# zertovitch/zip-ada

Hardware: AMD Instinct MI355X
Metric: Deflate encode MB/s (Deflate_3; stream bit-exact with the CPU restatement of the reference, Ada parity unpinned) (higher is better)
Workload: dtype u8

## Files before the change

### zip-ada_amd/csrc/zada_huff.hip

```cpp
#include <hip/hip_runtime.h>
#include <stdlib.h>
#include <stdio.h>
#include <stdint.h>
#include "zada_logic.h"
#include "zada_descr_bound.h"
#include "zada_internal.h"
#include "zada_llhc_wave.h"

namespace zada {

__device__ __forceinline__ void atom_symbols(uint32_t t, int &ls, int &ds) {
  if (tok_is_match(t)) { ls = len_symbol((int)((t >> 16) & 0x1FF)); ds = dist_symbol((int)(t & 0xFFFF)); }
  else { ls = (int)(t & 0xFF); ds = -1; }
}

__device__ __forceinline__ void put_bits_global(uint32_t *out32, uint64_t pos, uint32_t value, int nbits) {
  if (nbits <= 0) return;
  uint64_t w = pos >> 5; int sh = (int)(pos & 31);
  uint64_t v = (uint64_t)value << sh;
  atomicOr(&out32[w], (uint32_t)v);
  if (sh + nbits > 32) atomicOr(&out32[w + 1], (uint32_t)(v >> 32));
}

__device__ __forceinline__ void put_bits_lim(uint32_t *out32, uint64_t lim_bits, uint64_t pos, uint32_t value, int nbits) {
// ... 721 lines not shown
      const ChRec r = chrec[i];
      uint64_t rb = INF;
      if (T == BT_FIXED) rb = r.bits[0];
      else if (T == BT_DYNAMIC) {
        if (code_block == (int)i - 1) { if ((r.ok >> code_variant) & 1u) rb = r.bits[code_variant]; }
        else {
          const BlockInfo *bi = &binfo[i];
          const uint8_t *cl = code_block == CODE_CARRIED ? cin->bl : (code_variant == 1 ? binfo[code_block].bl1 : binfo[code_block].bl2);
          bool bad = false; uint64_t rc = 0;
          for (int q = 0; q < 5; q++) {
            const int s = lane + 64 * q;
            const int cu = cl[s]; const uint32_t stv = bi->stats[s];
            if (cu == 0 && bi->bl1[s] > 0) bad = true;
            if (s < 288) { if (s != 256 && s <= 285) rc += (uint64_t)stv * (uint64_t)(cu + litlen_sym_extra(s)); }
            else if (s - 288 <= 29) rc += (uint64_t)stv * (uint64_t)(cu + dist_sym_extra(s - 288));
          }
          rc = wave_sum_u64(rc);
          if (!__any(bad)) rb = rc;
        }
      }
      const bool finishing = B && (T == BT_FIXED || T == BT_DYNAMIC);
      const uint64_t c = 1 + (finishing ? (uint64_t)(eob >> 16) : 0);
      dec = ch_decide(r, c, rb);
      if (lane == 0) {
        ChW w; w.rdata = rb; w.eob_in = eob; w.dec = (uint8_t)dec; w.T_in = (uint8_t)T; w.B_in = (uint8_t)B; w.pad = 0;
        w.code_block = code_block; w.code_variant = (uint32_t)code_variant; w.npieces = 0; w.bytes_pad = 0;
        chw[i] = w;
      }
    } else dec = chw[i].dec;
    if (dec != FMT_RECYCLE) {
      uint32_t j = nblocks;
      for (uint32_t b0 = i + 1; b0 < nblocks && j == nblocks; b0 += 64) {
        const uint32_t k = b0 + (uint32_t)lane;
        const bool rcy = k < nblocks && chw[k].dec == FMT_RECYCLE;
        const unsigned long long m = __ballot(rcy);
        if (m) j = b0 + (uint32_t)(__ffsll((long long)m) - 1);
      }
      if (j == nblocks) break;
      out_state(j - 1);
      i = j; need_eval = false;
    } else {
      i++; need_eval = true;
    }
  }
}

template <typename F>
__device__ __forceinline__ uint32_t ch_stored_walk(const uint32_t *__restrict__ apos, uint32_t first, uint32_t count, uint32_t end_byte, int last_block, F &&piece) {
  uint32_t stk_first[40], stk_last[40]; int stk_lb[40]; int sp = 0;
  uint32_t np = 0;
  stk_first[0] = first; stk_last[0] = first + count - 1; stk_lb[0] = last_block; sp = 1;
  while (sp > 0) {
    sp--;
    const uint32_t f = stk_first[sp], l = stk_last[sp]; const int lb = stk_lb[sp];
    const uint32_t src = apos[f], nbytes = ((end_byte && l + 1 == first + count) ? end_byte : apos[l + 1]) - src;
    if (nbytes > 0xFFFF) {
      const uint32_t mid = (uint32_t)(((uint64_t)f + (uint64_t)l) / 2);
      stk_first[sp] = mid + 1; stk_last[sp] = l; stk_lb[sp] = lb; sp++;
      stk_first[sp] = f; stk_last[sp] = mid; stk_lb[sp] = 0; sp++;
      continue;
    }
    piece(np, src, nbytes, lb);
    np++;
  }
  return np;
}

__global__ void __launch_bounds__(64) k_ch_stored(uint32_t nblocks, const ChRec *__restrict__ chrec, const uint32_t *__restrict__ apos, ChW *__restrict__ chw) {
  const uint32_t i = blockIdx.x * blockDim.x + threadIdx.x;
  if (i >= nblocks || chw[i].dec != FMT_STORED) return;
  const BlockRange br = chrec[i].br;
  chw[i].npieces = ch_stored_walk(apos, br.first, br.count, br.pad, (int)(br.last_flush & BR_LAST_FLUSH), [](uint32_t, uint32_t, uint32_t, int) {});
}

struct PosFn { uint64_t a, b; uint32_t kind; };
__device__ __forceinline__ uint64_t posfn_apply(const PosFn &f, uint64_t p) { return f.kind == 2 ? f.b : f.kind ? ((p + f.a + 7) & ~7ull) + f.b : p + f.a; }
__device__ __forceinline__ PosFn posfn_compose(const PosFn &f, const PosFn &g) {
  PosFn h;
  if (g.kind == 2) return g;
  if (f.kind == 2) { h.kind = 2; h.a = 0; h.b = posfn_apply(g, f.b); return h; }
  if (g.kind == 0) { h.kind = f.kind; h.a = f.kind ? f.a : f.a + g.a; h.b = f.kind ? f.b + g.a : 0; }
  else if (f.kind == 0) { h.kind = 1; h.a = f.a + g.a; h.b = g.b; }
  else { h.kind = 1; h.a = f.a; h.b = ((f.b + g.a + 7) & ~7ull) + g.b; }
  return h;
}

__global__ void __launch_bounds__(1024) k_ch_layout(uint32_t nblocks, const ChRec *__restrict__ chrec, const BlockInfo *__restrict__ binfo, const ChW *__restrict__ chw,
                                                    EmitRec *__restrict__ emit, uint32_t *__restrict__ piece_base, uint32_t cap_tiles, uint32_t cap_pieces,
                                                    uint32_t *__restrict__ out32, uint64_t lim_bits, ChooserOut *__restrict__ res,
                                                    const ChooserCarry *__restrict__ cin, ChooserCarry *__restrict__ cout, uint64_t base_bits, int do_epilogue,
                                                    const uint32_t *__restrict__ blk_entry, EntOut *__restrict__ ent_out ) {
  __shared__ PosFn wfn[16];
  __shared__ uint32_t wtiles[16], wpieces[16], wlast[16];
  __shared__ uint64_t s_pos; __shared__ uint32_t s_tiles, s_pieces, s_last;
  const int tid = threadIdx.x, lane = tid & 63, w = tid >> 6;
  if (tid == 0) { s_pos = cin->pos - base_bits; s_tiles = 0; s_pieces = 0; s_last = 0xFFFFFFFFu; }
  __syncthreads();
  for (uint32_t t0 = 0; t0 < nblocks; t0 += 1024) {
    const uint32_t i = t0 + (uint32_t)tid;
    const bool ex = i < nblocks;
    PosFn f; f.kind = 0; f.a = 0; f.b = 0;
    uint32_t nt = 0, np = 0, opener = 0xFFFFFFFFu;
    ChRec r; ChW cw;
    uint64_t pre_bits = 0, hdr = 0, data = 0, opt = 0;
    bool opens = false;
    if (ex) {
      r = chrec[i]; cw = chw[i];
      const bool fin = cw.B_in && (cw.T_in == BT_FIXED || cw.T_in == BT_DYNAMIC);
      const uint64_t eobl = fin ? (uint64_t)(cw.eob_in >> 16) : 0;
      const uint64_t c = 1 + eobl;
      if (cw.dec == FMT_STORED) {
        np = cw.npieces;
        f.kind = 1; f.a = eobl + 3; f.b = 32ull * np + 8ull * (np - 1) + 8ull * binfo[i].bytes;
        opt = r.stored + c; opener = i;
      } else {
        nt = (r.br.count + TILE - 1) / TILE;
        if (cw.dec == FMT_RECYCLE) { data = cw.rdata; opt = cw.rdata; }
        else if (cw.dec == FMT_FIXED) { opens = cw.T_in != BT_FIXED; data = r.fixed_data; opt = r.base3 + c; }
        else { opens = true; hdr = cw.dec == FMT_DYN1 ? r.hdr1 : r.hdr2; data = cw.dec == FMT_DYN1 ? r.dyn1_data : r.dyn2_data; opt = r.base3 + c; }
        if (opens) { pre_bits = eobl + 3; opener = i; }
        f.a = pre_bits + hdr + data;
      }
    }
    const bool efirst = ex && ent_out && (r.br.last_flush & BR_ENTRY_FIRST), elast = ex && ent_out && (r.br.last_flush & BR_ENTRY_LAST);
    const PosFn fown = f;
    if (efirst) { f.kind = 2; f.a = 0; f.b = posfn_apply(fown, 0); }
    PosFn inc = f; uint32_t it = nt, ip = np, il = opener;
    for (int off = 1; off < 64; off <<= 1) {
      PosFn o; o.a = __shfl_up(inc.a, off); o.b = __shfl_up(inc.b, off); o.kind = __shfl_up(inc.kind, off);
      const uint32_t ot = __shfl_up(it, off), op = __shfl_up(ip, off), ol = __shfl_up(il, off);
      if (lane >= off) { inc = posfn_compose(o, inc); it += ot; ip += op; il = il == 0xFFFFFFFFu ? ol : il; }
    }
    if (lane == 63) { wfn[w] = inc; wtiles[w] = it; wpieces[w] = ip; }
    {
      const unsigned long long m = __ballot(opener != 0xFFFFFFFFu);
      if (lane == 0) wlast[w] = m ? t0 + (uint32_t)(w * 64 + 63 - __builtin_clzll(m)) : 0xFFFFFFFFu;
    }
    __syncthreads();
    PosFn before; before.kind = 0; before.a = 0; before.b = 0;
    uint32_t tb = 0, pb = 0;
    for (int k = 0; k < w; k++) { before = posfn_compose(before, wfn[k]); tb += wtiles[k]; pb += wpieces[k]; }
    PosFn exl; exl.a = __shfl_up(inc.a, 1); exl.b = __shfl_up(inc.b, 1); exl.kind = __shfl_up(inc.kind, 1);
    uint32_t ext = __shfl_up(it, 1), exp_ = __shfl_up(ip, 1);
    if (lane == 0) { exl.kind = 0; exl.a = 0; exl.b = 0; ext = 0; exp_ = 0; }
    const PosFn upto = posfn_compose(before, exl);
    const uint64_t p0 = efirst ? 0 : posfn_apply(upto, s_pos);
    const uint32_t tile0 = s_tiles + tb + ext, piece0 = s_pieces + pb + exp_;
    if (ex) {
      EmitRec e; e.hdr_bitpos = 0; e.data_bitpos = 0; e.cost_bits = opt; e.fmt = cw.dec; e.code_block = CODE_FIXED; e.code_variant = 0; e.tile_base = tile0;
      e.pre_pos = 0; e.pre_eob = 0; e.pre_flags = 0;
      if (cw.dec == FMT_STORED) {
        e.pre_pos = p0;
        e.pre_eob = (cw.B_in && (cw.T_in == BT_FIXED || cw.T_in == BT_DYNAMIC)) ? cw.eob_in : 0u;
        piece_base[i] = piece0;
      } else {
        if (opens) {
          e.pre_pos = p0;
          e.pre_eob = (cw.B_in && (cw.T_in == BT_FIXED || cw.T_in == BT_DYNAMIC)) ? cw.eob_in : 0u;
          e.pre_flags = 1u | ((r.br.last_flush & BR_LAST_FLUSH) << 1) | ((cw.dec == FMT_FIXED ? 1u : 2u) << 2);
        }
        e.hdr_bitpos = p0 + pre_bits;
        e.data_bitpos = p0 + pre_bits + hdr;
        if (cw.dec == FMT_RECYCLE || (cw.dec == FMT_FIXED && !opens)) { e.code_block = cw.code_block; e.code_variant = cw.code_variant; }
        else if (cw.dec == FMT_FIXED) { e.code_block = CODE_FIXED; e.code_variant = 0; }
        else { e.code_block = (int32_t)i; e.code_variant = cw.dec == FMT_DYN1 ? 1u : 2u; }
      }
      emit[i] = e;
      if (elast) {
        uint32_t lo = il;
        if (lo == 0xFFFFFFFFu) { for (int k = w - 1; k >= 0; k--) if (wlast[k] != 0xFFFFFFFFu) { lo = wlast[k]; break; } }
        if (lo == 0xFFFFFFFFu) lo = s_last;
        const uint32_t dk = chw[lo].dec;
        const ChRec rk = chrec[lo];
        EntOut eo; eo.bits = posfn_apply(fown, p0);
        eo.eob = dk == FMT_STORED ? 0u : dk == FMT_FIXED ? (7u << 16) : rk.eob[dk == FMT_DYN1 ? 0 : 1];
        eo.fake = (rk.br.last_flush & BR_LAST_FLUSH) ? 0u : 1u;
        ent_out[blk_entry[i]] = eo;
      }
    }
    __syncthreads();
    if (tid == 1023) {
      const PosFn all = posfn_compose(before, inc);
      s_pos = posfn_apply(all, s_pos); s_tiles += tb + it; s_pieces += pb + ip;
    }
    if (tid == 0) { for (int k = 15; k >= 0; k--) if (wlast[k] != 0xFFFFFFFFu) { s_last = wlast[k]; break; } }
    __syncthreads();
  }
  uint64_t pos = s_pos;
  int T = cin->last_type, B = cin->block_to_finish, M = cin->last_marked;
  uint32_t eob = cin->cur_eob;
  const uint8_t *cl = T == BT_DYNAMIC ? cin->bl : nullptr;
  if (s_last != 0xFFFFFFFFu) {
    const uint32_t k = s_last;
    const uint32_t dec = chw[k].dec;
    const ChRec r = chrec[k];
    B = 1; M = (int)(r.br.last_flush & BR_LAST_FLUSH); cl = nullptr;
    if (dec == FMT_STORED) T = BT_STORED;
    else if (dec == FMT_FIXED) { T = BT_FIXED; eob = 7u << 16; }
    else { T = BT_DYNAMIC; eob = r.eob[dec == FMT_DYN1 ? 0 : 1]; cl = dec == FMT_DYN1 ? binfo[k].bl1 : binfo[k].bl2; }
    if (dec == FMT_STORED) eob = chw[k].eob_in;
  }
  if (do_epilogue) {
    if (B && (T == BT_FIXED || T == BT_DYNAMIC)) {
      if (tid == 0) put_bits_lim(out32, lim_bits, pos, eob & 0xFFFF, (int)(eob >> 16));
      pos += (uint64_t)(eob >> 16);
    }
    if (!M) {
      if (tid == 0) { put_bits_lim(out32, lim_bits, pos, 1, 1); put_bits_lim(out32, lim_bits, pos + 1, 1, 2); }
      pos += 3 + 7;
    }
  }
  if (tid < 320) cout->bl[tid] = cl ? cl[tid] : (uint8_t)0;
  if (tid == 0) {
    res->total_bits = pos; res->n_tiles = s_tiles; res->n_pieces = s_pieces; res->n_blocks = nblocks;
    res->overflow = (s_tiles > cap_tiles || s_pieces > cap_pieces) ? 1u : 0u;
    cout->pos = pos + base_bits; cout->last_type = T; cout->block_to_finish = B; cout->last_marked = M; cout->cur_eob = eob; cout->pad[0] = cout->pad[1] = 0;
  }
}

__global__ void k_batch_geom(uint32_t E, const uint32_t *__restrict__ chunk0, const uint32_t *__restrict__ fl0, const uint32_t *__restrict__ ent_start,
                             const uint32_t *__restrict__ ent_len, const uint32_t *__restrict__ offsets, const uint32_t *__restrict__ total_atoms,
                             FlushGeom *__restrict__ ftab, EntOut *__restrict__ ent_out) {
  const uint32_t e = blockIdx.x * blockDim.x + threadIdx.x;
  if (e >= E) return;
  const uint32_t a0 = offsets[chunk0[e]], a1 = e + 1 < E ? offsets[chunk0[e + 1]] : *total_atoms, T = a1 - a0;
  const uint32_t nfl = (T + FLUSH - 1) / FLUSH;
  for (uint32_t s = fl0[e], k = 0; s < fl0[e + 1]; s++, k++) {
    FlushGeom g; g.F = a0 + k * FLUSH; g.to = 0; g.gj = k; g.flags = FG_EMPTY; g.end_byte = ent_start[e] + ent_len[e]; g.entry = e; g.pad[0] = g.pad[1] = 0;
    if (k < nfl) {
      g.to = g.F + FLUSH - 1 < a1 - 1 ? g.F + FLUSH - 1 : a1 - 1;
      g.flags = (k == 0 ? (uint32_t)FG_ENTRY_FIRST : 0u) | (k + 1 == nfl ? (uint32_t)FG_ENTRY_LAST : 0u) |
                ((k + 1 == nfl && (T % FLUSH) != 0) ? (uint32_t)FG_LAST_PARTIAL : 0u);
    }
    ftab[s] = g;
  }
  EntOut eo; eo.bits = 0; eo.eob = 0; eo.fake = 1;
  ent_out[e] = eo;
}

__global__ void k_batch_sizes(uint32_t E, const EntOut *__restrict__ ent_out, uint32_t *__restrict__ ent_bytes) {
  const uint32_t e = blockIdx.x * blockDim.x + threadIdx.x;
  if (e >= E) return;
  const EntOut eo = ent_out[e];
  ent_bytes[e] = (uint32_t)((eo.bits + (eo.eob >> 16) + (eo.fake ? 10u : 0u) + 7) / 8);
}

__global__ void k_batch_rebase(uint32_t nblocks, const uint32_t *__restrict__ blk_entry, const uint32_t *__restrict__ ent_base, EmitRec *__restrict__ emit) {
  const uint32_t i = blockIdx.x * blockDim.x + threadIdx.x;
  if (i >= nblocks) return;
  const uint64_t b = 8ull * ent_base[blk_entry[i]];
  emit[i].hdr_bitpos += b; emit[i].data_bitpos += b; emit[i].pre_pos += b;
}

__global__ void k_batch_finish(uint32_t E, const EntOut *__restrict__ ent_out, const uint32_t *__restrict__ ent_base, uint32_t *__restrict__ out32, uint64_t lim_bits) {
  const uint32_t e = blockIdx.x * blockDim.x + threadIdx.x;
  if (e >= E) return;
  const EntOut eo = ent_out[e];
  uint64_t pos = 8ull * ent_base[e] + eo.bits;
  if (eo.eob) { put_bits_lim(out32, lim_bits, pos, eo.eob & 0xFFFF, (int)(eo.eob >> 16)); pos += eo.eob >> 16; }
  if (eo.fake) { put_bits_lim(out32, lim_bits, pos, 1, 1); put_bits_lim(out32, lim_bits, pos + 1, 1, 2); }
}

__global__ void __launch_bounds__(64) k_ch_stored_emit(uint32_t nblocks, const ChRec *__restrict__ chrec, const ChW *__restrict__ chw, const EmitRec *__restrict__ emit,
                                                       const uint32_t *__restrict__ piece_base, const uint32_t *__restrict__ apos,
                                                       StoredPiece *__restrict__ pieces, uint32_t *__restrict__ out32, uint64_t lim_bits) {
  const uint32_t i = blockIdx.x * blockDim.x + threadIdx.x;
  if (i >= nblocks || chw[i].dec != FMT_STORED) return;
  const BlockRange br = chrec[i].br;
  const EmitRec e = emit[i];
  uint64_t pos = e.pre_pos;
  const uint32_t pb = piece_base[i];
  bool first = true;
  ch_stored_walk(apos, br.first, br.count, br.pad, (int)(br.last_flush & BR_LAST_FLUSH), [&](uint32_t k, uint32_t src, uint32_t nbytes, int lb) {
    if (first && e.pre_eob) { put_bits_lim(out32, lim_bits, pos, e.pre_eob & 0xFFFF, (int)(e.pre_eob >> 16)); pos += e.pre_eob >> 16; }
    first = false;
    put_bits_lim(out32, lim_bits, pos, (uint32_t)lb, 1);
    pos += 3;
    pos = (pos + 7) & ~7ull;
    put_bits_lim(out32, lim_bits, pos, nbytes & 0xFFFF, 16);
    put_bits_lim(out32, lim_bits, pos + 16, (~nbytes) & 0xFFFF, 16);
    StoredPiece pc; pc.dst_byte = (pos >> 3) + 4; pc.src_byte = src; pc.nbytes = nbytes;
    pieces[pb + k] = pc;
    pos += 32 + 8ull * nbytes;
  });
}

__global__ void __launch_bounds__(256) k_emit_prefix(uint32_t nblocks, const EmitRec *__restrict__ emit, const BlockRange *__restrict__ blocks,
                                                     uint32_t *__restrict__ tile_block, uint32_t *__restrict__ out32) {
  const uint32_t i = blockIdx.x * blockDim.x + threadIdx.x;
  if (i >= nblocks) return;
  const EmitRec e = emit[i];
  if (e.pre_flags & 1u) {
    uint64_t p = e.pre_pos;
    if (e.pre_eob) { put_bits_global(out32, p, e.pre_eob & 0xFFFF, (int)(e.pre_eob >> 16)); p += e.pre_eob >> 16; }
    put_bits_global(out32, p, (e.pre_flags >> 1) & 1u, 1);
    put_bits_global(out32, p + 1, (e.pre_flags >> 2) & 3u, 2);
  }
  if (e.fmt != FMT_STORED) {
    const uint32_t nt = (blocks[i].count + TILE - 1) / TILE;
    for (uint32_t t = 0; t < nt; t++) tile_block[e.tile_base + t] = i;
  }
}

__global__ void __launch_bounds__(64) k_block_codes(uint32_t nblocks, const EmitRec *__restrict__ emit, const BlockInfo *__restrict__ binfo,
                                                    uint32_t *__restrict__ codes, const ChooserCarry *__restrict__ cin) {
  __shared__ uint8_t bl[320];
  __shared__ uint16_t cd[320];
  const uint32_t b = blockIdx.x;
  const int lane = threadIdx.x;
  if (b == nblocks) {
    for (int i = lane; i < 320; i += 64) bl[i] = (uint8_t)(i < 288 ? fixed_litlen_bl(i) : 5);
  } else if (b == nblocks + 1) {
    for (int i = lane; i < 320; i += 64) bl[i] = cin->bl[i];
  } else {
    const uint32_t f = emit[b].fmt;
    if (f != FMT_DYN1 && f != FMT_DYN2) return;
    const uint8_t *src = f == FMT_DYN1 ? binfo[b].bl1 : binfo[b].bl2;
    for (int i = lane; i < 320; i += 64) bl[i] = src[i];
  }
  __syncthreads();
  if (lane == 0) canonical_codes(bl, 288, cd);
  if (lane == 1) canonical_codes(bl + 288, 32, cd + 288);
  __syncthreads();
  for (int i = lane; i < 320; i += 64) codes[(uint64_t)b * 320 + i] = ((uint32_t)bl[i] << 16) | cd[i];
}

__device__ __forceinline__ uint32_t code_table_index(const EmitRec &e, uint32_t nblocks) {
  return e.code_block == CODE_FIXED ? nblocks : (e.code_block == CODE_CARRIED ? nblocks + 1 : (uint32_t)e.code_block);
}

__device__ __forceinline__ int atom_bits(uint32_t t, const uint32_t *tab, uint64_t &v) {
  if (!tok_is_match(t)) { uint32_t c = tab[t & 0xFF]; v = c & 0xFFFF; return (int)(c >> 16); }
  const int len = (int)((t >> 16) & 0x1FF), dist = (int)(t & 0xFFFF);
  uint32_t lc = tab[len_symbol(len)], dc = tab[288 + dist_symbol(dist)];
  int n = (int)(lc >> 16);
  v = lc & 0xFFFF;
  int le = len_extra_bits(len);
  v |= (uint64_t)len_extra_val(len) << n; n += le;
  v |= (uint64_t)(dc & 0xFFFF) << n; n += (int)(dc >> 16);
  int de = dist_extra_bits(dist);
  v |= (uint64_t)dist_extra_val(dist) << n; n += de;
  return n;
}

__global__ void __launch_bounds__(256) k_tile_bits(uint32_t nblocks, const uint32_t *__restrict__ atoms, const BlockRange *__restrict__ blocks,
                                                   const EmitRec *__restrict__ emit, const uint32_t *__restrict__ tile_block,
                                                   const uint32_t *__restrict__ codes, uint32_t *__restrict__ tile_bits) {
  __shared__ uint32_t tab[320];
  __shared__ uint32_t red[4];
  const uint32_t t = blockIdx.x, b = tile_block[t];
  const EmitRec e = emit[b];
  const BlockRange br = blocks[b];
  const uint32_t ti = t - e.tile_base;
  const uint32_t a0 = br.first + ti * TILE, a1 = (ti * TILE + TILE < br.count) ? a0 + TILE : br.first + br.count;
  const uint32_t *src = codes + (uint64_t)code_table_index(e, nblocks) * 320;
  const int tid = threadIdx.x;
  for (int i = tid; i < 320; i += 256) tab[i] = src[i];
  __syncthreads();
  uint32_t s = 0;
  for (uint32_t a = a0 + tid; a < a1; a += 256) { uint64_t v; s += (uint32_t)atom_bits(atoms[a], tab, v); }
  s = wave_sum_u32(s);
  if ((tid & 63) == 0) red[tid >> 6] = s;
  __syncthreads();
  if (tid == 0) tile_bits[t] = red[0] + red[1] + red[2] + red[3];
}

__global__ void k_tile_scan(uint32_t nblocks, const BlockRange *__restrict__ blocks, const EmitRec *__restrict__ emit,
                            const uint32_t *__restrict__ tile_bits, uint64_t *__restrict__ tile_bitpos) {
  uint32_t b = blockIdx.x * blockDim.x + threadIdx.x;
  if (b >= nblocks) return;
  const EmitRec e = emit[b];
  if (e.fmt == FMT_STORED) return;
  uint32_t nt = (blocks[b].count + TILE - 1) / TILE;
  uint64_t pos = e.data_bitpos;
  for (uint32_t t = 0; t < nt; t++) { tile_bitpos[e.tile_base + t] = pos; pos += tile_bits[e.tile_base + t]; }
}

__global__ void __launch_bounds__(256) k_emit_tiles(uint32_t nblocks, const uint32_t *__restrict__ atoms, const BlockRange *__restrict__ blocks,
                                                    const EmitRec *__restrict__ emit, const uint32_t *__restrict__ tile_block,
                                                    const uint32_t *__restrict__ codes, const uint64_t *__restrict__ tile_bitpos,
                                                    uint32_t *__restrict__ out32) {
  __shared__ uint32_t tab[320];
  __shared__ uint32_t buf[TILE * 48 / 32 + 4];
  __shared__ uint32_t wsum[4];
  const uint32_t t = blockIdx.x, b = tile_block[t];
  const EmitRec e = emit[b];
  const BlockRange br = blocks[b];
  const uint32_t ti = t - e.tile_base;
  const uint32_t a0 = br.first + ti * TILE, a1 = (ti * TILE + TILE < br.count) ? a0 + TILE : br.first + br.count;
  const uint32_t *src = codes + (uint64_t)code_table_index(e, nblocks) * 320;
  const int tid = threadIdx.x, lane = tid & 63, w = tid >> 6;
  for (int i = tid; i < 320; i += 256) tab[i] = src[i];
  for (int i = tid; i < (int)(TILE * 48 / 32 + 4); i += 256) buf[i] = 0;
  __syncthreads();
  uint64_t v[8]; int nb[8]; uint32_t tot = 0;
  for (int k = 0; k < 8; k++) {
    uint32_t a = a0 + tid * 8 + k;
    if (a < a1) { nb[k] = atom_bits(atoms[a], tab, v[k]); tot += (uint32_t)nb[k]; } else { nb[k] = 0; v[k] = 0; }
  }
  uint32_t incl = tot;
  for (int off = 1; off < 64; off <<= 1) { uint32_t x = __shfl_up(incl, off); if (lane >= off) incl += x; }
  if (lane == 63) wsum[w] = incl;
  __syncthreads();
  uint32_t base = 0;
  for (int k = 0; k < w; k++) base += wsum[k];
  const uint64_t b0 = tile_bitpos[t];
  uint32_t bp = (uint32_t)(b0 & 31) + base + incl - tot;
  for (int k = 0; k < 8; k++) {
    if (nb[k]) {
      uint32_t wd = bp >> 5; int sh = (int)(bp & 31);
      uint64_t lo = v[k] << sh;
      atomicOr(&buf[wd], (uint32_t)lo);
      if (sh + nb[k] > 32) atomicOr(&buf[wd + 1], (uint32_t)(lo >> 32));
      if (sh + nb[k] > 64) atomicOr(&buf[wd + 2], (uint32_t)(v[k] >> (64 - sh)));
      bp += (uint32_t)nb[k];
    }
  }
  __syncthreads();
  const uint32_t tile_total = wsum[0] + wsum[1] + wsum[2] + wsum[3];
  const uint32_t nwords = ((uint32_t)(b0 & 31) + tile_total + 31) >> 5;
  uint32_t *dst = out32 + (b0 >> 5);
  for (uint32_t i = tid; i < nwords; i += 256) {
    uint32_t x = buf[i];
    if (i == 0 || i + 1 == nwords) { if (x) atomicOr(&dst[i], x); }
    else dst[i] = x;
  }
}

__global__ void __launch_bounds__(64) k_emit_headers(uint32_t nblocks, const EmitRec *__restrict__ emit, const BlockInfo *__restrict__ binfo,
                                                     uint32_t *__restrict__ out32) {
  __shared__ uint8_t bl[320], cs[320], tbl[20];
  __shared__ uint16_t tcode[19];
  const uint32_t b = blockIdx.x;
  const EmitRec e = emit[b];
  if (e.fmt != FMT_DYN1 && e.fmt != FMT_DYN2) return;
  const int lane = threadIdx.x;
  const BlockInfo *bi = &binfo[b];
  const uint8_t *src = e.fmt == FMT_DYN1 ? bi->bl1 : bi->bl2;
  const uint8_t *tsrc = e.fmt == FMT_DYN1 ? bi->truc1 : bi->truc2;
  for (int i = lane; i < 320; i += 64) bl[i] = src[i];
  if (lane < 20) tbl[lane] = tsrc[lane];
  __syncthreads();
  if (lane != 0) return;
  int max_ll = 0, max_d = 0, n = 0;
  for (int a = 287; a >= 0; a--) if (bl[a] > 0) { max_ll = a; break; }
  for (int a = 31; a >= 0; a--) if (bl[288 + a] > 0) { max_d = a; break; }
  for (int a = 0; a <= max_ll; a++) cs[n++] = bl[a];
  for (int a = 0; a <= max_d; a++) cs[n++] = bl[288 + a];
  canonical_codes(tbl, 19, tcode);
  const int anz = tbl[19];
  uint64_t pos = e.hdr_bitpos;
  put_bits_global(out32, pos, (uint32_t)(max_ll - 256), 5); pos += 5;
  put_bits_global(out32, pos, (uint32_t)max_d, 5); pos += 5;
  put_bits_global(out32, pos, (uint32_t)(anz - 3), 4); pos += 4;
  for (int a = 0; a <= anz; a++) { put_bits_global(out32, pos, tbl[header_perm(a)], 3); pos += 3; }
  header_rle_walk(cs, n, [&](int x, uint32_t extra) {
    put_bits_global(out32, pos, tcode[x], tbl[x]); pos += tbl[x];
    int eb = header_extra_bits(x);
    if (eb) { put_bits_global(out32, pos, extra, eb); pos += eb; }
  });
}

__global__ void __launch_bounds__(256) k_copy_pieces(uint32_t npieces, const StoredPiece *__restrict__ pieces,
                                                     const uint8_t *__restrict__ in, uint8_t *__restrict__ out) {
  const uint32_t p = blockIdx.x;
  if (p >= npieces) return;
  const StoredPiece pc = pieces[p];
  for (uint32_t i = blockIdx.y * 256 + threadIdx.x; i < pc.nbytes; i += gridDim.y * 256) out[pc.dst_byte + i] = in[(uint64_t)pc.src_byte + i];
}

__global__ void k_set_u32(uint32_t *p, uint32_t v) { if (threadIdx.x == 0 && blockIdx.x == 0) *p = v; }

static EntropyView range_view(Ctx *c) {
  const Range &R = c->rg;
  Workspace &W = c->ws;
  EntropyView v;
  v.ftab = R.batch ? W.ftab : nullptr;
  v.atoms = W.ea_atoms + (LB_CAP - R.n_lb); v.apos = W.ea_apos + (LB_CAP - R.n_lb);
  const uint64_t tv = R.T_view == ~0ull ? R.T : R.T_view;
  v.foff = R.foff; v.nflush = R.nflush; v.lvalid = (uint32_t)(R.n_lb + tv + R.n_la);
  v.stream_final = (R.G + tv + R.n_la == R.T_total) ? 1u : 0u;
  v.j0 = R.j0;
  return v;
}

int batch_geometry(Ctx *c, uint32_t E, const uint32_t *d_total_atoms) {
  Workspace &W = c->ws;
  hipLaunchKernelGGL(k_batch_geom, dim3((E + 255) / 256), dim3(256), 0, c->stream, E, W.ent_chunk0, W.ent_fl0, W.ent_start, W.ent_len, W.offsets,
                     d_total_atoms, W.ftab, W.ent_out);
  return hip_check(c, hipGetLastError(), "batch_geometry");
}

int entropy_analyze(Ctx *c) {
  hipStream_t st = c->stream;
  Workspace &W = c->ws;
  Range &R = c->rg;
  const bool fixed_only = (R.method == 6);
  const EntropyView v = range_view(c);
  uint32_t nblocks = 0;
  hipLaunchKernelGGL(k_apos_sentinel, dim3(1), dim3(1), 0, st, v.atoms, (uint32_t *)v.apos, v.lvalid);
  if (v.nflush > 0) {
    if (fixed_only && !R.batch) {
      nblocks = v.nflush;
      hipLaunchKernelGGL(k_fill_blocks_fixed, dim3((nblocks + 255) / 256), dim3(256), 0, st, v.foff, v.lvalid - v.foff, nblocks, W.blocks);
    } else {
      const uint32_t kstep = fixed_only ? (1u << 30) : R.method == 8 ? 8 : R.method == 9 ? 4 : 1;
      const bool lazy = kstep == 1 && c->knob_descr_lazy;
      uint32_t cnt[3] = {0, 0, 0};
      if (lazy) {
        hipMemsetAsync(W.descr_cnt, 0, 3 * 4, st);
        hipLaunchKernelGGL(k_piece_masks, dim3(v.nflush * PM_GROUPS), dim3(256), 0, st, v, W.pmask);
        hipLaunchKernelGGL(k_window_descr, dim3(v.nflush * WD_NGROUPS), dim3(64), 0, st, v, 4u, W.descr);
      } else if (!fixed_only) hipLaunchKernelGGL(k_window_descr, dim3(v.nflush * WD_NGROUPS), dim3(64), 0, st, v, kstep, W.descr);
      c->tmark("window_descr");
      if (lazy) hipLaunchKernelGGL(k_cut_scan_lazy, dim3(v.nflush), dim3(64), 0, st, v, W.descr, W.pmask, W.seg_nblk, W.seg_cut, W.descr_cnt);
      else hipLaunchKernelGGL(k_cut_scan, dim3(v.nflush), dim3(64), 0, st, v, kstep, W.descr, W.seg_nblk, W.seg_cut, W.cut_trace);
      c->trace_stale = lazy;
      exclusive_scan_u32(st, W.seg_nblk, W.seg_blk_off, W.scan2, W.total2, v.nflush);
      hipMemcpyAsync(&nblocks, W.total2, 4, hipMemcpyDeviceToHost, st);
      if (lazy) hipMemcpyAsync(cnt, W.descr_cnt, 3 * 4, hipMemcpyDeviceToHost, st);
      hipLaunchKernelGGL(k_fill_blocks, dim3((v.nflush + 255) / 256), dim3(256), 0, st, v, W.seg_nblk, W.seg_cut, W.seg_blk_off, W.blocks, W.blk_entry, fixed_only ? 1 : 0);
      if (hip_check(c, hipStreamSynchronize(st), "cut_scan")) return ZADA_E_HIP_;
      c->tmark("cut_scan");
      c->descr_l3 += cnt[0]; c->descr_excluded += cnt[1]; c->descr_late += cnt[2];
    }
    if (nblocks > W.cap_blocks) { c->err = "block table overflow"; return -1; }
    if (nblocks > 0) hipLaunchKernelGGL(k_block_analyze, dim3(nblocks), dim3(256), 0, st, v.atoms, v.apos, W.blocks, W.binfo);
    c->tmark("block_analyze");
#ifdef ZADA_BA_STATS
    { unsigned long long h[16]; hipDeviceSynchronize(); hipMemcpyFromSymbol(h, HIP_SYMBOL(g_ba_dbg), sizeof h);
      const double nb = h[8] ? (double)h[8] : 1.0;
      fprintf(stderr, "[k_block_analyze] %llu blocks, %.0f atoms per block; cycles per block: histogram %.0f, tweaks %.0f, patches %.0f, codings %.0f, header plan %.0f, header code %.0f, "
              "a_non_zero + bits %.0f, costs + output %.0f\n", h[8], (double)h[9] / nb, (double)h[0] / nb, (double)h[1] / nb, (double)h[2] / nb, (double)h[3] / nb, (double)h[4] / nb, (double)h[5] / nb,
              (double)h[6] / nb, (double)h[7] / nb);
      for (int q = 0; q < 16; q++) h[q] = 0;
      hipMemcpyToSymbol(HIP_SYMBOL(g_ba_dbg), h, sizeof h); }
#endif
    if ((!fixed_only || R.batch) && nblocks > 0) hipLaunchKernelGGL(k_block_relate, dim3(nblocks), dim3(64), 0, st, nblocks, W.binfo, W.blocks, (ChRec *)W.chrec);
  }
  R.nblocks = nblocks;
  R.analyzed = true;
  return hip_check(c, hipGetLastError(), "entropy_analyze");
}

int entropy_trace(Ctx *c) {
  if (!c->trace_stale) return 0;
  const Range &R = c->rg;
  Workspace &W = c->ws;
  if (!R.analyzed || R.method == 6 || R.nflush == 0) return 0;
  const EntropyView v = range_view(c);
  const uint32_t kstep = R.method == 8 ? 8 : R.method == 9 ? 4 : 1;
  hipLaunchKernelGGL(k_window_descr, dim3(v.nflush * WD_NGROUPS), dim3(64), 0, c->stream, v, kstep, W.descr);
  hipLaunchKernelGGL(k_cut_scan, dim3(v.nflush), dim3(64), 0, c->stream, v, kstep, W.descr, W.seg_nblk, W.seg_cut, W.cut_trace);
  if (hip_check(c, hipGetLastError(), "trace")) return ZADA_E_HIP_;
  c->trace_stale = false;
  return 0;
}

int entropy_choose(Ctx *c) {
  hipStream_t st = c->stream;
  Workspace &W = c->ws;
  Range &R = c->rg;
  const bool fixed_only = (R.method == 6);
  const EntropyView v = range_view(c);
  if (R.batch) { R.carry_in = ChooserCarry(); R.carry_in.last_type = BT_RESERVED; R.carry_in.cur_eob = 7u << 16; }
  R.base_bits = R.carry_in.pos & ~7ull;
  hipMemcpyAsync(W.carry, &R.carry_in, sizeof(ChooserCarry), hipMemcpyHostToDevice, st);
  const uint64_t lim_bits = W.cap_out * 8;
  if (fixed_only && !R.batch)
    hipLaunchKernelGGL(k_choose_fixed, dim3(1), dim3(64), 0, st, R.nblocks, W.blocks, W.binfo, W.emit, W.tile_block, (uint32_t)W.cap_tiles,
                       (uint32_t *)W.out, lim_bits, W.chooser, W.carry, W.carry + 1, R.base_bits, R.G == 0 ? 1 : 0, v.stream_final ? 1 : 0);
  else {
    const int do_epilogue = !R.batch && v.stream_final && (v.nflush > 0 || R.T_total == 0);
    const uint32_t nb = R.nblocks;
    ChW *chw = (ChW *)W.chw;
    if (nb > 0) {
      hipLaunchKernelGGL(k_ch_tentative, dim3((nb + 255) / 256), dim3(256), 0, st, nb, (const ChRec *)W.chrec, chw, fixed_only ? 1 : 0);
      if (!fixed_only) hipLaunchKernelGGL(k_ch_resolve, dim3(1), dim3(64), 0, st, nb, (const ChRec *)W.chrec, W.binfo, chw, W.carry, R.batch ? 1 : 0);
      hipLaunchKernelGGL(k_ch_stored, dim3((nb + 63) / 64), dim3(64), 0, st, nb, (const ChRec *)W.chrec, v.apos, chw);
    }
    hipLaunchKernelGGL(k_ch_layout, dim3(1), dim3(1024), 0, st, nb, (const ChRec *)W.chrec, W.binfo, chw, W.emit, W.piece_base,
                       (uint32_t)W.cap_tiles, (uint32_t)W.cap_pieces, (uint32_t *)W.out, lim_bits, W.chooser, W.carry, W.carry + 1, R.base_bits, do_epilogue,
                       W.blk_entry, R.batch ? W.ent_out : nullptr);
    if (R.batch) {
      const uint32_t E = R.n_entries;
      hipLaunchKernelGGL(k_batch_sizes, dim3((E + 255) / 256), dim3(256), 0, st, E, W.ent_out, W.ent_bytes);
      exclusive_scan_u32(st, W.ent_bytes, W.ent_base, W.scan2, W.total2, E);
      if (nb > 0) hipLaunchKernelGGL(k_batch_rebase, dim3((nb + 255) / 256), dim3(256), 0, st, nb, W.blk_entry, W.ent_base, W.emit);
      hipLaunchKernelGGL(k_batch_finish, dim3((E + 255) / 256), dim3(256), 0, st, E, W.ent_out, W.ent_base, (uint32_t *)W.out, lim_bits);
    }
  }
  uint32_t batch_bytes = 0;
  if (R.batch) hipMemcpyAsync(&batch_bytes, W.total2, 4, hipMemcpyDeviceToHost, st);
  hipMemcpyAsync(&R.co, W.chooser, sizeof(ChooserOut), hipMemcpyDeviceToHost, st);
  hipMemcpyAsync(&R.carry_out, W.carry + 1, sizeof(ChooserCarry), hipMemcpyDeviceToHost, st);
  if (hip_check(c, hipStreamSynchronize(st), "choose")) return ZADA_E_HIP_;
  c->tmark("choose");
  if (R.co.overflow) { c->err = "emission table overflow"; return -1; }
  if (R.batch) R.co.total_bits = 8ull * batch_bytes;
  R.chosen = true;
  c->last_nblocks = R.nblocks;
  return 0;
}

int entropy_emit(Ctx *c, uint8_t *d_out) {
  hipStream_t st = c->stream;
  Workspace &W = c->ws;
  Range &R = c->rg;
  const bool fixed_only = (R.method == 6);
  const uint32_t nblocks = R.nblocks;
  const ChooserOut &co = R.co;
  if ((co.total_bits + 7) / 8 + 8 > W.cap_out) { c->err = "output workspace overflow"; return -1; }
  if ((!fixed_only || R.batch) && nblocks > 0)
    hipLaunchKernelGGL(k_emit_prefix, dim3((nblocks + 255) / 256), dim3(256), 0, st, nblocks, W.emit, W.blocks, W.tile_block, (uint32_t *)W.out);
  hipLaunchKernelGGL(k_block_codes, dim3(nblocks + 2), dim3(64), 0, st, nblocks, W.emit, W.binfo, W.codes, W.carry);
  const EntropyView v = range_view(c);
  if (co.n_tiles > 0) {
    hipLaunchKernelGGL(k_tile_bits, dim3(co.n_tiles), dim3(256), 0, st, nblocks, v.atoms, W.blocks, W.emit, W.tile_block, W.codes, W.tile_bits);
    hipLaunchKernelGGL(k_tile_scan, dim3((nblocks + 255) / 256), dim3(256), 0, st, nblocks, W.blocks, W.emit, W.tile_bits, W.tile_bitpos);
    hipLaunchKernelGGL(k_emit_tiles, dim3(co.n_tiles), dim3(256), 0, st, nblocks, v.atoms, W.blocks, W.emit, W.tile_block, W.codes, W.tile_bitpos, (uint32_t *)W.out);
  }
  if (nblocks > 0 && !fixed_only) hipLaunchKernelGGL(k_emit_headers, dim3(nblocks), dim3(64), 0, st, nblocks, W.emit, W.binfo, (uint32_t *)W.out);
  if (co.n_pieces > 0) {
    hipLaunchKernelGGL(k_ch_stored_emit, dim3((nblocks + 63) / 64), dim3(64), 0, st, nblocks, (const ChRec *)W.chrec, (const ChW *)W.chw, W.emit, W.piece_base, v.apos,
                       W.pieces, (uint32_t *)W.out, W.cap_out * 8);
    hipLaunchKernelGGL(k_copy_pieces, dim3(co.n_pieces, 16), dim3(256), 0, st, co.n_pieces, W.pieces, R.rin, W.out);
  }
  if (d_out) hipMemcpyAsync(d_out, W.out, (co.total_bits + 7) / 8, hipMemcpyDeviceToDevice, st);
  c->tmark("emit");
  return hip_check(c, hipGetLastError(), "entropy_emit");
}

}
```

Baseline: 9755.

## Merge header emission into wave-parallel block table kernel and vectorize atom loads

Replaces the serial single-lane canonical code and header emission with a wave-parallel version using ballots and prefix scans, and fuses header writing into the code-table kernel so one launch is dropped. The header is assembled in an LDS image and flushed as whole words. k_tile_bits now reads a byte-length table and loads atoms with 16-byte vector loads, and k_emit_tiles loads eight atoms with two wide loads and splits each atom's bits into two 32-bit parts. Optional cycle-stat instrumentation is added behind a compile flag. The parallel run/RLE planning is more complex and must stay bit-exact with the serial walk.

```diff
diff --git a/zip-ada_amd/csrc/zada_huff.hip b/zip-ada_amd/csrc/zada_huff.hip
--- a/zip-ada_amd/csrc/zada_huff.hip
+++ b/zip-ada_amd/csrc/zada_huff.hip
@@ -1047,51 +1047,193 @@
   }
 }
 
-__global__ void __launch_bounds__(64) k_block_codes(uint32_t nblocks, const EmitRec *__restrict__ emit, const BlockInfo *__restrict__ binfo,
-                                                    uint32_t *__restrict__ codes, const ChooserCarry *__restrict__ cin) {
-  __shared__ uint8_t bl[320];
-  __shared__ uint16_t cd[320];
+#ifdef ZADA_EM_STATS
+__device__ unsigned long long g_em_dbg[16];
+#define EM_BEGIN() unsigned long long em_t = clock64()
+#define EM_STAMP(k) do { if (threadIdx.x == 0) { const unsigned long long t_ = clock64(); atomicAdd(&g_em_dbg[k], t_ - em_t); em_t = t_; } } while (0)
+#define EM_COUNT(k) do { if (threadIdx.x == 0) atomicAdd(&g_em_dbg[k], 1ull); } while (0)
+#else
+#define EM_BEGIN() do { } while (0)
+#define EM_STAMP(k) do { } while (0)
+#define EM_COUNT(k) do { } while (0)
+#endif
+
+__device__ __forceinline__ void canonical_codes_wave(const int (&l)[5], uint32_t (&code)[5], int lane) {
+  const unsigned long long below = (1ull << lane) - 1;
+  uint32_t nc_ll = 0, nc_d = 0, cnt_ll = 0, cnt_d = 0;
+#pragma unroll
+  for (int r = 0; r < 5; r++) code[r] = 0;
+  for (int len = 1; len <= 15; len++) {
+    nc_ll = (nc_ll + cnt_ll) << 1; nc_d = (nc_d + cnt_d) << 1;
+    cnt_ll = 0; cnt_d = 0;
+#pragma unroll
+    for (int r = 0; r < 4; r++) {
+      const unsigned long long m = __ballot(l[r] == len);
+      if (l[r] == len) code[r] = nc_ll + cnt_ll + (uint32_t)__popcll(m & below);
+      cnt_ll += (uint32_t)__popcll(m);
+    }
+    const unsigned long long m = __ballot(l[4] == len), ml = m & 0xFFFFFFFFull, md = m >> 32;
+    if (l[4] == len) code[4] = lane < 32 ? nc_ll + cnt_ll + (uint32_t)__popcll(ml & below) : nc_d + (uint32_t)__popcll(md & (below >> 32));
+    cnt_ll += (uint32_t)__popcll(ml); cnt_d = (uint32_t)__popcll(md);
+  }
+#pragma unroll
+  for (int r = 0; r < 5; r++) code[r] = l[r] ? (__brev(code[r]) >> (32 - l[r])) & 0xFFFFu : 0u;
+}
+
+template <typename Sink>
+__device__ __forceinline__ void header_run_walk(int v, int len, Sink &&sink) {
+  for (int k = 0; k < len;) {
+    int rep = len - k;
+    if (k > 0 && rep >= 3 && !(v == 0 && rep > 6)) { rep = rep < 6 ? rep : 6; sink(16, (uint32_t)(rep - 3)); k += rep; }
+    else if (v == 0 && rep >= 3) {
+      if (rep <= 10) sink(17, (uint32_t)(rep - 3));
+      else { rep = rep < 138 ? rep : 138; sink(18, (uint32_t)(rep - 11)); }
+      k += rep;
+    } else { sink(v, 0u); k++; }
+  }
+}
+
+constexpr int HDR_IMG_WORDS = 76;
+__device__ __forceinline__ void img_put(uint32_t *img, uint32_t pos, uint32_t value, int nbits) {
+  const uint32_t wd = pos >> 5; const int sh = (int)(pos & 31);
+  const uint64_t v = (uint64_t)value << sh;
+  atomicOr(&img[wd], (uint32_t)v);
+  if (sh + nbits > 32) atomicOr(&img[wd + 1], (uint32_t)(v >> 32));
+}
+
+__global__ void __launch_bounds__(64) k_block_tables(uint32_t nblocks, const EmitRec *__restrict__ emit, const BlockInfo *__restrict__ binfo,
+                                                     uint32_t *__restrict__ codes, const ChooserCarry *__restrict__ cin, uint32_t *__restrict__ out32) {
+  __shared__ uint8_t bl[320], tbl[20];
+  __shared__ uint32_t tcl[19], img[HDR_IMG_WORDS];
+  __shared__ uint64_t map[5];
   const uint32_t b = blockIdx.x;
   const int lane = threadIdx.x;
+  EM_BEGIN();
+  bool dyn = false;
+  EmitRec e;
   if (b == nblocks) {
     for (int i = lane; i < 320; i += 64) bl[i] = (uint8_t)(i < 288 ? fixed_litlen_bl(i) : 5);
   } else if (b == nblocks + 1) {
     for (int i = lane; i < 320; i += 64) bl[i] = cin->bl[i];
   } else {
-    const uint32_t f = emit[b].fmt;
-    if (f != FMT_DYN1 && f != FMT_DYN2) return;
-    const uint8_t *src = f == FMT_DYN1 ? binfo[b].bl1 : binfo[b].bl2;
+    e = emit[b];
+    if (e.fmt != FMT_DYN1 && e.fmt != FMT_DYN2) return;
+    dyn = true;
+    const BlockInfo *bi = &binfo[b];
+    const uint8_t *src = e.fmt == FMT_DYN1 ? bi->bl1 : bi->bl2;
+    const uint8_t *tsrc = e.fmt == FMT_DYN1 ? bi->truc1 : bi->truc2;
     for (int i = lane; i < 320; i += 64) bl[i] = src[i];
-  }
-  __syncthreads();
-  if (lane == 0) canonical_codes(bl, 288, cd);
-  if (lane == 1) canonical_codes(bl + 288, 32, cd + 288);
-  __syncthreads();
-  for (int i = lane; i < 320; i += 64) codes[(uint64_t)b * 320 + i] = ((uint32_t)bl[i] << 16) | cd[i];
+    if (lane < 20) tbl[lane] = tsrc[lane];
+    for (int i = lane; i < HDR_IMG_WORDS; i += 64) img[i] = 0;
+  }
+  wave_sync();
+  EM_STAMP(0);
+  int l[5]; uint32_t code[5];
+#pragma unroll
+  for (int r = 0; r < 5; r++) l[r] = bl[lane + 64 * r];
+  canonical_codes_wave(l, code, lane);
+  EM_STAMP(4);
+#pragma unroll
+  for (int r = 0; r < 5; r++) codes[(uint64_t)b * 320 + lane + 64 * r] = ((uint32_t)l[r] << 16) | code[r];
+  EM_STAMP(5); EM_COUNT(12);
+  if (!dyn) return;
+  const unsigned long long below = (1ull << lane) - 1;
+  int max_ll = 0;
+#pragma unroll
+  for (int r = 0; r < 5; r++) {
+    const unsigned long long m = __ballot(l[r] > 0 && (r < 4 || lane < 32));
+    if (m) max_ll = 64 * r + 63 - __builtin_clzll(m);
+  }
+  const unsigned long long dm = __ballot(l[4] > 0 && lane >= 32) >> 32;
+  const int max_d = dm ? 63 - __builtin_clzll(dm) : 0;
+  const int n = max_ll + 1 + max_d + 1;
+  {
+    const int tl = lane < 19 ? tbl[lane] : 0;
+    uint32_t tc = 0, nc = 0, cnt = 0;
+    for (int len = 1; len <= 15; len++) {
+      nc = (nc + cnt) << 1;
+      const unsigned long long m = __ballot(tl == len);
+      if (tl == len) tc = nc + (uint32_t)__popcll(m & below);
+      cnt = (uint32_t)__popcll(m);
+    }
+    if (lane < 19) tcl[lane] = ((uint32_t)tl << 16) | (tl ? (__brev(tc) >> (32 - tl)) & 0xFFFFu : 0u);
+  }
+  int cv[5]; bool start[5];
+#pragma unroll
+  for (int r = 0; r < 5; r++) {
+    const int i = lane + 64 * r;
+    cv[r] = i < n ? (int)(i <= max_ll ? bl[i] : bl[288 + i - max_ll - 1]) : -1;
+    const int pv = (i > 0 && i < n) ? (int)(i - 1 <= max_ll ? bl[i - 1] : bl[288 + i - 1 - max_ll - 1]) : -2;
+    start[r] = i < n && cv[r] != pv;
+    const unsigned long long m = __ballot(start[r] || i == n);
+    if (lane == 0) map[r] = m;
+  }
+  wave_sync();
+  const int anz = tbl[19];
+  const uint32_t sh0 = (uint32_t)(e.hdr_bitpos & 31), fixed_bits = 14u + 3u * (uint32_t)(anz + 1);
+  int rl[5]; uint32_t off[5], carry = sh0 + fixed_bits;
+#pragma unroll
+  for (int r = 0; r < 5; r++) {
+    uint32_t x = 0;
+    rl[r] = 0;
+    if (start[r]) {
+      const int i = lane + 64 * r;
+      rl[r] = posmap_next(map, i) - i;
+      header_run_walk(cv[r], rl[r], [&](int s, uint32_t) { x += (tcl[s] >> 16) + (uint32_t)header_extra_bits(s); });
+    }
+    uint32_t incl = x;
+    for (int o = 1; o < 64; o <<= 1) { const uint32_t y = __shfl_up(incl, o); if (lane >= o) incl += y; }
+    off[r] = carry + incl - x;
+    carry += __shfl(incl, 63);
+  }
+  EM_STAMP(1);
+  if (lane == 0) img_put(img, sh0, (uint32_t)(max_ll - 256) | ((uint32_t)max_d << 5) | ((uint32_t)(anz - 3) << 10), 14);
+  if (lane <= anz) img_put(img, sh0 + 14u + 3u * (uint32_t)lane, tbl[header_perm(lane < 19 ? lane : 0)], 3);
+#pragma unroll
+  for (int r = 0; r < 5; r++) {
+    if (start[r]) {
+      uint32_t pos = off[r];
+      header_run_walk(cv[r], rl[r], [&](int s, uint32_t extra) {
+        const uint32_t c = tcl[s]; const int cl = (int)(c >> 16), nb = cl + header_extra_bits(s);
+        img_put(img, pos, (c & 0xFFFFu) | (extra << cl), nb);
+        pos += (uint32_t)nb;
+      });
+    }
+  }
+  wave_sync();
+  const uint32_t nwords = (carry + 31) >> 5;
+  uint32_t *dst = out32 + (e.hdr_bitpos >> 5);
+  for (uint32_t i = lane; i < nwords; i += 64) {
+    const uint32_t x = img[i];
+    if (i == 0 || i + 1 == nwords) { if (x) atomicOr(&dst[i], x); }
+    else dst[i] = x;
+  }
+  EM_STAMP(2); EM_COUNT(11);
 }
 
 __device__ __forceinline__ uint32_t code_table_index(const EmitRec &e, uint32_t nblocks) {
   return e.code_block == CODE_FIXED ? nblocks : (e.code_block == CODE_CARRIED ? nblocks + 1 : (uint32_t)e.code_block);
 }
 
-__device__ __forceinline__ int atom_bits(uint32_t t, const uint32_t *tab, uint64_t &v) {
-  if (!tok_is_match(t)) { uint32_t c = tab[t & 0xFF]; v = c & 0xFFFF; return (int)(c >> 16); }
+__device__ __forceinline__ uint32_t atom_len_bits(uint32_t t, const uint8_t *lens) {
+  if (!tok_is_match(t)) return lens[t & 0xFF];
   const int len = (int)((t >> 16) & 0x1FF), dist = (int)(t & 0xFFFF);
-  uint32_t lc = tab[len_symbol(len)], dc = tab[288 + dist_symbol(dist)];
-  int n = (int)(lc >> 16);
-  v = lc & 0xFFFF;
-  int le = len_extra_bits(len);
-  v |= (uint64_t)len_extra_val(len) << n; n += le;
-  v |= (uint64_t)(dc & 0xFFFF) << n; n += (int)(dc >> 16);
-  int de = dist_extra_bits(dist);
-  v |= (uint64_t)dist_extra_val(dist) << n; n += de;
-  return n;
+  return (uint32_t)lens[len_symbol(len)] + (uint32_t)len_extra_bits(len) + (uint32_t)lens[288 + dist_symbol(dist)] + (uint32_t)dist_extra_bits(dist);
+}
+
+__device__ __forceinline__ void atom_parts(uint32_t t, const uint32_t *tab, uint32_t &a, int &na, uint32_t &d, int &nd) {
+  if (!tok_is_match(t)) { const uint32_t c = tab[t & 0xFF]; a = c & 0xFFFF; na = (int)(c >> 16); d = 0; nd = 0; return; }
+  const int len = (int)((t >> 16) & 0x1FF), dist = (int)(t & 0xFFFF);
+  const uint32_t lc = tab[len_symbol(len)], dc = tab[288 + dist_symbol(dist)];
+  const int nl = (int)(lc >> 16), nc = (int)(dc >> 16);
+  a = (lc & 0xFFFF) | (len_extra_val(len) << nl); na = nl + len_extra_bits(len);
+  d = (dc & 0xFFFF) | (dist_extra_val(dist) << nc); nd = nc + dist_extra_bits(dist);
 }
 
 __global__ void __launch_bounds__(256) k_tile_bits(uint32_t nblocks, const uint32_t *__restrict__ atoms, const BlockRange *__restrict__ blocks,
                                                    const EmitRec *__restrict__ emit, const uint32_t *__restrict__ tile_block,
                                                    const uint32_t *__restrict__ codes, uint32_t *__restrict__ tile_bits) {
-  __shared__ uint32_t tab[320];
+  __shared__ uint8_t tab[320];
   __shared__ uint32_t red[4];
   const uint32_t t = blockIdx.x, b = tile_block[t];
   const EmitRec e = emit[b];
@@ -1100,10 +1242,21 @@
   const uint32_t a0 = br.first + ti * TILE, a1 = (ti * TILE + TILE < br.count) ? a0 + TILE : br.first + br.count;
   const uint32_t *src = codes + (uint64_t)code_table_index(e, nblocks) * 320;
   const int tid = threadIdx.x;
-  for (int i = tid; i < 320; i += 256) tab[i] = src[i];
+  for (int i = tid; i < 320; i += 256) tab[i] = (uint8_t)(src[i] >> 16);
   __syncthreads();
+  const uint32_t *p = atoms + a0;
+  const uint32_t na = a1 - a0;
+  uint32_t head = (uint32_t)((16u - ((uintptr_t)p & 15u)) & 15u) >> 2;
+  if (head > na) head = na;
+  const uint32_t nq = (na - head) >> 2, tail = head + 4 * nq;
+  const uint4 *q = (const uint4 *)(p + head);
   uint32_t s = 0;
-  for (uint32_t a = a0 + tid; a < a1; a += 256) { uint64_t v; s += (uint32_t)atom_bits(atoms[a], tab, v); }
+  if ((uint32_t)tid < head) s += atom_len_bits(p[tid], tab);
+  for (uint32_t i = tid; i < nq; i += 256) {
+    const uint4 x = q[i];
+    s += atom_len_bits(x.x, tab) + atom_len_bits(x.y, tab) + atom_len_bits(x.z, tab) + atom_len_bits(x.w, tab);
+  }
+  if (tail + tid < na) s += atom_len_bits(p[tail + tid], tab);
   s = wave_sum_u32(s);
   if ((tid & 63) == 0) red[tid >> 6] = s;
   __syncthreads();
@@ -1120,6 +1273,8 @@
   uint64_t pos = e.data_bitpos;
   for (uint32_t t = 0; t < nt; t++) { tile_bitpos[e.tile_base + t] = pos; pos += tile_bits[e.tile_base + t]; }
 }
+
+struct __attribute__((packed, aligned(4))) Atoms4 { uint32_t x, y, z, w; };
 
 __global__ void __launch_bounds__(256) k_emit_tiles(uint32_t nblocks, const uint32_t *__restrict__ atoms, const BlockRange *__restrict__ blocks,
                                                     const EmitRec *__restrict__ emit, const uint32_t *__restrict__ tile_block,
@@ -1135,14 +1290,27 @@
   const uint32_t a0 = br.first + ti * TILE, a1 = (ti * TILE + TILE < br.count) ? a0 + TILE : br.first + br.count;
   const uint32_t *src = codes + (uint64_t)code_table_index(e, nblocks) * 320;
   const int tid = threadIdx.x, lane = tid & 63, w = tid >> 6;
+  EM_BEGIN();
   for (int i = tid; i < 320; i += 256) tab[i] = src[i];
   for (int i = tid; i < (int)(TILE * 48 / 32 + 4); i += 256) buf[i] = 0;
   __syncthreads();
-  uint64_t v[8]; int nb[8]; uint32_t tot = 0;
+  EM_STAMP(6);
+  uint32_t va[8], vd[8], nn[8], tot = 0;
+  const uint32_t al = a0 + tid * 8, nv = al >= a1 ? 0u : (a1 - al < 8u ? a1 - al : 8u);
+  uint32_t at[8];
+  if (nv == 8) {
+    const Atoms4 q0 = *(const Atoms4 *)(atoms + al), q1 = *(const Atoms4 *)(atoms + al + 4);
+    at[0] = q0.x; at[1] = q0.y; at[2] = q0.z; at[3] = q0.w; at[4] = q1.x; at[5] = q1.y; at[6] = q1.z; at[7] = q1.w;
+  } else {
+#pragma unroll
+    for (int k = 0; k < 8; k++) at[k] = (uint32_t)k < nv ? atoms[al + k] : 0u;
+  }
+#pragma unroll
   for (int k = 0; k < 8; k++) {
-    uint32_t a = a0 + tid * 8 + k;
-    if (a < a1) { nb[k] = atom_bits(atoms[a], tab, v[k]); tot += (uint32_t)nb[k]; } else { nb[k] = 0; v[k] = 0; }
-  }
+    va[k] = 0; vd[k] = 0; nn[k] = 0;
+    if ((uint32_t)k < nv) { int na, nd; atom_parts(at[k], tab, va[k], na, vd[k], nd); nn[k] = (uint32_t)na | ((uint32_t)nd << 8); tot += (uint32_t)(na + nd); }
+  }
+  EM_STAMP(7);
   uint32_t incl = tot;
   for (int off = 1; off < 64; off <<= 1) { uint32_t x = __shfl_up(incl, off); if (lane >= off) incl += x; }
   if (lane == 63) wsum[w] = incl;
@@ -1151,17 +1319,22 @@
   for (int k = 0; k < w; k++) base += wsum[k];
   const uint64_t b0 = tile_bitpos[t];
   uint32_t bp = (uint32_t)(b0 & 31) + base + incl - tot;
+  EM_STAMP(8);
+#pragma unroll
   for (int k = 0; k < 8; k++) {
-    if (nb[k]) {
+    const int na = (int)(nn[k] & 0xFF), nb = na + (int)(nn[k] >> 8);
+    if (nb) {
+      const uint64_t v = (uint64_t)va[k] | ((uint64_t)vd[k] << na);
       uint32_t wd = bp >> 5; int sh = (int)(bp & 31);
-      uint64_t lo = v[k] << sh;
+      uint64_t lo = v << sh;
       atomicOr(&buf[wd], (uint32_t)lo);
-      if (sh + nb[k] > 32) atomicOr(&buf[wd + 1], (uint32_t)(lo >> 32));
-      if (sh + nb[k] > 64) atomicOr(&buf[wd + 2], (uint32_t)(v[k] >> (64 - sh)));
-      bp += (uint32_t)nb[k];
+      if (sh + nb > 32) atomicOr(&buf[wd + 1], (uint32_t)(lo >> 32));
+      if (sh + nb > 64) atomicOr(&buf[wd + 2], (uint32_t)(v >> (64 - sh)));
+      bp += (uint32_t)nb;
     }
   }
   __syncthreads();
+  EM_STAMP(9);
   const uint32_t tile_total = wsum[0] + wsum[1] + wsum[2] + wsum[3];
   const uint32_t nwords = ((uint32_t)(b0 & 31) + tile_total + 31) >> 5;
   uint32_t *dst = out32 + (b0 >> 5);
@@ -1170,40 +1343,7 @@
     if (i == 0 || i + 1 == nwords) { if (x) atomicOr(&dst[i], x); }
     else dst[i] = x;
   }
-}
-
-__global__ void __launch_bounds__(64) k_emit_headers(uint32_t nblocks, const EmitRec *__restrict__ emit, const BlockInfo *__restrict__ binfo,
-                                                     uint32_t *__restrict__ out32) {
-  __shared__ uint8_t bl[320], cs[320], tbl[20];
-  __shared__ uint16_t tcode[19];
-  const uint32_t b = blockIdx.x;
-  const EmitRec e = emit[b];
-  if (e.fmt != FMT_DYN1 && e.fmt != FMT_DYN2) return;
-  const int lane = threadIdx.x;
-  const BlockInfo *bi = &binfo[b];
-  const uint8_t *src = e.fmt == FMT_DYN1 ? bi->bl1 : bi->bl2;
-  const uint8_t *tsrc = e.fmt == FMT_DYN1 ? bi->truc1 : bi->truc2;
-  for (int i = lane; i < 320; i += 64) bl[i] = src[i];
-  if (lane < 20) tbl[lane] = tsrc[lane];
-  __syncthreads();
-  if (lane != 0) return;
-  int max_ll = 0, max_d = 0, n = 0;
-  for (int a = 287; a >= 0; a--) if (bl[a] > 0) { max_ll = a; break; }
-  for (int a = 31; a >= 0; a--) if (bl[288 + a] > 0) { max_d = a; break; }
-  for (int a = 0; a <= max_ll; a++) cs[n++] = bl[a];
-  for (int a = 0; a <= max_d; a++) cs[n++] = bl[288 + a];
-  canonical_codes(tbl, 19, tcode);
-  const int anz = tbl[19];
-  uint64_t pos = e.hdr_bitpos;
-  put_bits_global(out32, pos, (uint32_t)(max_ll - 256), 5); pos += 5;
-  put_bits_global(out32, pos, (uint32_t)max_d, 5); pos += 5;
-  put_bits_global(out32, pos, (uint32_t)(anz - 3), 4); pos += 4;
-  for (int a = 0; a <= anz; a++) { put_bits_global(out32, pos, tbl[header_perm(a)], 3); pos += 3; }
-  header_rle_walk(cs, n, [&](int x, uint32_t extra) {
-    put_bits_global(out32, pos, tcode[x], tbl[x]); pos += tbl[x];
-    int eb = header_extra_bits(x);
-    if (eb) { put_bits_global(out32, pos, extra, eb); pos += eb; }
-  });
+  EM_STAMP(10); EM_COUNT(13);
 }
 
 __global__ void __launch_bounds__(256) k_copy_pieces(uint32_t npieces, const StoredPiece *__restrict__ pieces,
@@ -1358,14 +1498,13 @@
   if ((co.total_bits + 7) / 8 + 8 > W.cap_out) { c->err = "output workspace overflow"; return -1; }
   if ((!fixed_only || R.batch) && nblocks > 0)
     hipLaunchKernelGGL(k_emit_prefix, dim3((nblocks + 255) / 256), dim3(256), 0, st, nblocks, W.emit, W.blocks, W.tile_block, (uint32_t *)W.out);
-  hipLaunchKernelGGL(k_block_codes, dim3(nblocks + 2), dim3(64), 0, st, nblocks, W.emit, W.binfo, W.codes, W.carry);
+  hipLaunchKernelGGL(k_block_tables, dim3(nblocks + 2), dim3(64), 0, st, nblocks, W.emit, W.binfo, W.codes, W.carry, (uint32_t *)W.out);
   const EntropyView v = range_view(c);
   if (co.n_tiles > 0) {
     hipLaunchKernelGGL(k_tile_bits, dim3(co.n_tiles), dim3(256), 0, st, nblocks, v.atoms, W.blocks, W.emit, W.tile_block, W.codes, W.tile_bits);
     hipLaunchKernelGGL(k_tile_scan, dim3((nblocks + 255) / 256), dim3(256), 0, st, nblocks, W.blocks, W.emit, W.tile_bits, W.tile_bitpos);
     hipLaunchKernelGGL(k_emit_tiles, dim3(co.n_tiles), dim3(256), 0, st, nblocks, v.atoms, W.blocks, W.emit, W.tile_block, W.codes, W.tile_bitpos, (uint32_t *)W.out);
   }
-  if (nblocks > 0 && !fixed_only) hipLaunchKernelGGL(k_emit_headers, dim3(nblocks), dim3(64), 0, st, nblocks, W.emit, W.binfo, (uint32_t *)W.out);
   if (co.n_pieces > 0) {
     hipLaunchKernelGGL(k_ch_stored_emit, dim3((nblocks + 63) / 64), dim3(64), 0, st, nblocks, (const ChRec *)W.chrec, (const ChW *)W.chw, W.emit, W.piece_base, v.apos,
                        W.pieces, (uint32_t *)W.out, W.cap_out * 8);
@@ -1373,6 +1512,15 @@
   }
   if (d_out) hipMemcpyAsync(d_out, W.out, (co.total_bits + 7) / 8, hipMemcpyDeviceToDevice, st);
   c->tmark("emit");
+#ifdef ZADA_EM_STATS
+  { unsigned long long h[16]; hipDeviceSynchronize(); hipMemcpyFromSymbol(h, HIP_SYMBOL(g_em_dbg), sizeof h);
+    const double nh = h[11] ? (double)h[11] : 1.0, nc = h[12] ? (double)h[12] : 1.0, nt = h[13] ? (double)h[13] : 1.0;
+    fprintf(stderr, "[emit] %llu headers, cycles per block: staging %.0f, plan %.0f, output %.0f; %llu code tables, cycles per table: staging %.0f, codes %.0f, output %.0f; "
+            "%llu tiles, cycles per tile: table staging %.0f, atom bits %.0f, prefix %.0f, LDS words %.0f, flush %.0f\n", h[11], (double)h[0] / nh, (double)h[1] / nh, (double)h[2] / nh,
+            h[12], (double)h[3] / nc, (double)h[4] / nc, (double)h[5] / nc, h[13], (double)h[6] / nt, (double)h[7] / nt, (double)h[8] / nt, (double)h[9] / nt, (double)h[10] / nt);
+    for (int q = 0; q < 16; q++) h[q] = 0;
+    hipMemcpyToSymbol(HIP_SYMBOL(g_em_dbg), h, sizeof h); }
+#endif
   return hip_check(c, hipGetLastError(), "entropy_emit");
 }
 
```

Result: no change. 9850, median of 6 (+1.0%).
